# Somedaywilldo/BM-NAS

Measured on AMD Instinct MI355X. Metric: search-steps/sec (fwd+bwd of fusion hypernet) on MM-IMDB synthetic, higher is better.
Workload: dtype f32; 1 GPU; mmimdb fusion search, batch 128 per GPU x 1 GPU(s), N6 C192 L16 steps2 node_steps1 node_multiplier1, train mode, dropout 0.1/0.1(attn); inputs=(b, C, L) features, global_batch=128, per_gpu_batch=128, parallelism=dp1, mode=graph, step=fwd+bwd, one hipGraph replay

## Files before the change

### bm-nas_amd/csrc/arch_body.hpp

```cpp
#pragma once
#include "common.hpp"

namespace {

struct ArchPack {
  const float* a[BMNAS_MAX_PTRS];
  const float* b[BMNAS_MAX_PTRS];
  float* o[BMNAS_MAX_PTRS];
  int rows[BMNAS_MAX_PTRS], cols[BMNAS_MAX_PTRS];
  int n, n_shards;
  int64_t shard_stride;
};

__device__ __forceinline__ void arch_softmax_bwd_row(const ArchPack& P, int r, int lane) {
  const int col = lane & 3, sg = lane >> 2;
  for (int t = 0; t < P.n; ++t) {
    if (r < P.rows[t]) {
      const int cols = P.cols[t];
      float dw = 0.f, w = 0.f;
      if (col < cols) {
        const float* dwp = P.b[t] + r * cols + col;
        for (int sh = sg; sh < P.n_shards; sh += 16) dw += dwp[(int64_t)sh * P.shard_stride];
        w = P.a[t][r * cols + col];
      }
      dw = row_stride4_sum(dw);
      dw = xor16_sum(dw);
      dw = xor32_sum(dw);
      float dot = w * dw;
      dot += lane_xor1(dot);
      dot += lane_xor2(dot);
      if (sg == 0 && col < cols) P.o[t][r * cols + col] = w * (dw - dot);
      return;
    }
    r -= P.rows[t];
  }
}

inline int fill_arch_pack(ArchPack& P, const float* const* a, const float* const* dw, float* const* out,
                          const int* rows, const int* cols, int n, int backward, int n_shards,
                          int64_t shard_stride) {
  if (!a || !out || !rows || !cols || n < 1 || (backward && !dw) || n_shards < 1) return BMNAS_E_ARG;
  if (n > BMNAS_MAX_PTRS) return BMNAS_E_LIMIT;
  int total = 0;
  for (int t = 0; t < n; ++t) {
    if (!a[t] || !out[t] || rows[t] < 1 || cols[t] < 1 || cols[t] > 4 || (backward && !dw[t]))
      return BMNAS_E_ARG;
    P.a[t] = a[t];
    P.b[t] = backward ? dw[t] : nullptr;
    P.o[t] = out[t];
    P.rows[t] = rows[t];
    P.cols[t] = cols[t];
    total += rows[t];
  }
  P.n = n;
  P.n_shards = n_shards;
  P.shard_stride = shard_stride;
  return total;
}

}
```

### bm-nas_amd/csrc/bnmix.hip

```cpp
#include "common.hpp"
#include "../../include/bmnas_hip.h"
#include "arch_body.hpp"
#include "bn_fin.hpp"
#include "mix_common.hpp"
#include "mish.hpp"
#include <algorithm>
#include <cstdlib>

namespace {

constexpr float kEps = 1e-5f;
constexpr float kMomentum = 0.1f;

__global__ __launch_bounds__(256) void bn_finalize_k(const float* __restrict__ part, int n_part,
                                                     int b, int L, int M,
                                                     const float* __restrict__ bn_w,
                                                     const float* __restrict__ bn_b,
                                                     float* running_mean, float* running_var,
                                                     int64_t* nbt, int n_nbt, int training,
                                                     float* __restrict__ chan) {
  const int lane = threadIdx.x & 63;
  const int m = blockIdx.x * 4 + (threadIdx.x >> 6);
  if (m >= M) return;
  float mean, rstd;
// ... 1058 lines not shown
  float* Weff[kMaxFold];
  int n, M, C, blocks_per;
};

__device__ __forceinline__ void cell_prologue_body(const ArchPack& P, const FoldPack& F,
                                                   unsigned long long* step_counter,
                                                   const unsigned long long* step_span,
                                                   float* __restrict__ scrub, int64_t scrub4, const int bid,
                                                   const int nblocks) {
  const int nfb = F.n * F.blocks_per;
  for (int64_t i = (int64_t)bid * 256 + threadIdx.x; i < scrub4; i += (int64_t)nblocks * 256)
    st4_wt(scrub + 4 * i, make_float4(0.f, 0.f, 0.f, 0.f));
  if (step_counter != nullptr && bid == nblocks - 1 && threadIdx.x == 0)
    step_counter[0] += step_span[0];
  if (bid < nfb) {
    const int q = bid / F.blocks_per, bi = bid - q * F.blocks_per;
    const float* __restrict__ W = F.W[q];
    float* __restrict__ We = F.Weff[q];
    const int c4n = F.C / 4;
    const int total = F.M * c4n;
    for (int i = bi * 256 + threadIdx.x; i < total; i += F.blocks_per * 256) {
      const int m = i / c4n, c4 = i - m * c4n;
      const float* r = W + (int64_t)m * 2 * F.C + 4 * c4;
      st4_wt(We + (int64_t)m * F.C + 4 * c4, f4_add(ld4(r), ld4(r + F.C)));
    }
    return;
  }
  int r = (bid - nfb) * 256 + threadIdx.x;
  for (int t = 0; t < P.n; ++t) {
    if (r < P.rows[t]) {
      const int cols = P.cols[t];
      const float* a = P.a[t] + r * cols;
      float* o = P.o[t] + r * cols;
      float mx = a[0];
      for (int p = 1; p < cols; ++p) mx = fmaxf(mx, a[p]);
      float den = 0.f;
      for (int p = 0; p < cols; ++p) den += expf(a[p] - mx);
      for (int p = 0; p < cols; ++p) o[p] = expf(a[p] - mx) / den;
      return;
    }
    r -= P.rows[t];
  }
}

__global__ __launch_bounds__(256) void cell_prologue_k(ArchPack P, FoldPack F, unsigned long long* step_counter,
                                                       const unsigned long long* step_span,
                                                       float* __restrict__ scrub, int64_t scrub4) {
  cell_prologue_body(P, F, step_counter, step_span, scrub, scrub4, (int)blockIdx.x, (int)gridDim.x);
}

__device__ __forceinline__ float softmax2_col1(const float* a) {
  const float a0 = a[0], a1 = a[1];
  const float mx = fmaxf(a0, a1);
  const float e0 = expf(a0 - mx), e1 = expf(a1 - mx);
  return e1 / (e0 + e1);
}

struct PairArgs {
  PtrsIn xs;
  const float* alpha;
  const float* beta;
  float* out;
  float* out2;
  int64_t n4;
};

template <int NIN>
__global__ __launch_bounds__(256) void cell_prologue_pair_k(ArchPack P, FoldPack F, unsigned long long* step_counter,
                                                            const unsigned long long* step_span,
                                                            float* __restrict__ scrub, int64_t scrub4, int n_pro,
                                                            PairArgs A) {
  if ((int)blockIdx.x < n_pro) {
    cell_prologue_body(P, F, step_counter, step_span, scrub, scrub4, (int)blockIdx.x, n_pro);
    return;
  }
  float wj[NIN];
#pragma unroll
  for (int j = 0; j < NIN; ++j) wj[j] = softmax2_col1(A.alpha + 2 * j);
  const float s2 = softmax2_col1(A.beta) + softmax2_col1(A.beta + 2);
  const int64_t stride = (int64_t)(gridDim.x - n_pro) * 256;
  for (int64_t i = (int64_t)(blockIdx.x - n_pro) * 256 + threadIdx.x; i < A.n4; i += stride) {
    float4 v[NIN];
#pragma unroll
    for (int j = 0; j < NIN; ++j) v[j] = reinterpret_cast<const float4*>(A.xs.p[j])[i];
    float4 acc = f4_scale(v[0], wj[0]);
#pragma unroll
    for (int j = 1; j < NIN; ++j) {
      acc.x = fmaf(wj[j], v[j].x, acc.x);
      acc.y = fmaf(wj[j], v[j].y, acc.y);
      acc.z = fmaf(wj[j], v[j].z, acc.z);
      acc.w = fmaf(wj[j], v[j].w, acc.w);
    }
    st4_w0<0>(A.out + 4 * i, acc);
    st4_w0<0>(A.out2 + 4 * i, f4_scale(acc, s2));
  }
}

}

extern "C" int bmnas_version(void) { return 100; }

extern "C" int bmnas_bn_finalize(const float* part, int n_part, int b, int L, int M,
                                 const float* bn_w, const float* bn_b, float* running_mean,
                                 float* running_var, int64_t* num_batches_tracked, int n_nbt,
                                 int training, float* chan, void* stream) {
  if (!bn_w || !bn_b || !chan || M < 1 || b < 1 || L < 1) return BMNAS_E_ARG;
  if (training && (!part || n_part < 1 || b * L < 2)) return BMNAS_E_ARG;
  if (!training && (!running_mean || !running_var)) return BMNAS_E_ARG;
  hipLaunchKernelGGL(bn_finalize_k, dim3((M + 3) / 4), dim3(256), 0, (hipStream_t)stream, part,
                     n_part, b, L, M, bn_w, bn_b, running_mean, running_var, num_batches_tracked,
                     n_nbt, training, chan);
  BMNAS_CHECK_LAUNCH();
  return 0;
}

extern "C" int bmnas_node_mix_fwd_next(const float* x, const float* y, const float* p1, const float* U,
                                       float* chan, bmnas_bn_fin_t fin, const float* gamma, float* out,
                                       int b, int C, int L, bmnas_dropout_t drop_glu,
                                       bmnas_dropout_t drop_fc, const float* const* prev, int n_prev,
                                       const float* w, int w_stride, float* z_next, void* stream) {
  if (!x || !y || !p1 || !U || !chan || !gamma || !out || b < 0 || C < 1 || n_prev < 0) return BMNAS_E_ARG;
  if (L % 4 || L > 16) return BMNAS_E_SHAPE;
  if (n_prev > kMixPrev) return BMNAS_E_LIMIT;
  MixNextF N{};
  if (n_prev > 0) {
    if (!prev || !w || !z_next || w_stride < 1) return BMNAS_E_ARG;
    for (int j = 0; j < n_prev; ++j) {
// ... 618 lines not shown
```

### bm-nas_amd/csrc/common.hpp

```cpp
#pragma once
#include <hip/hip_runtime.h>
#include <stdint.h>

#define BMNAS_MAX_PTRS 16
#define BMNAS_WAVE 64

typedef __attribute__((ext_vector_type(4))) float f32x4;

struct PtrsIn { const float* p[BMNAS_MAX_PTRS]; };
struct PtrsOut { float* p[BMNAS_MAX_PTRS]; };

struct DropCfg {
  uint32_t thr;
  float scale;
  uint64_t seed;
  uint64_t offset;
  const uint64_t* step;
};

#define BMNAS_CHECK_LAUNCH()                         \
  do {                                               \
    hipError_t e__ = hipGetLastError();              \
    if (e__ != hipSuccess) return (int)e__;          \
  } while (0)
// ... 212 lines not shown
  float t = red[0];
#pragma unroll
  for (int k = 1; k < NW; ++k) t += red[k];
  v[0] = t;
  if (threadIdx.x == 0) {
#pragma unroll
    for (int i = 1; i < N; ++i) {
      float u = red[i * NW];
#pragma unroll
      for (int k = 1; k < NW; ++k) u += red[i * NW + k];
      v[i] = u;
    }
  }
}

template <typename T>
__device__ __forceinline__ T* sgpr_ptr(T* p) {
  asm volatile("" : "+s"(p));
  return p;
}
template <typename T, int N>
__device__ __forceinline__ T* pick_ptr(T* const (&arr)[N], int q) {
  T* p = sgpr_ptr(arr[0]);
#pragma unroll
  for (int qq = 1; qq < N; ++qq) {
    T* c = sgpr_ptr(arr[qq]);
    p = (q == qq) ? c : p;
  }
  return p;
}

__device__ __forceinline__ float4 ld4(const float* p) { return *reinterpret_cast<const float4*>(p); }
__device__ __forceinline__ void st4(float* p, float4 v) { *reinterpret_cast<float4*>(p) = v; }
__device__ __forceinline__ void st4_wt(float* p, float4 v) {
#if defined(BMNAS_NO_WT)
  *reinterpret_cast<float4*>(p) = v;
#else
  const f32x4 d = {v.x, v.y, v.z, v.w};
  asm volatile("global_store_dwordx4 %0, %1, off sc1\n\ts_nop 1" : : "v"(p), "v"(d) : "memory");
#endif
}

#ifndef BMNAS_WT_MASK
#define BMNAS_WT_MASK 0x29
#endif
template <int G>
__device__ __forceinline__ void st4_wtg(float* p, float4 v) {
  if constexpr ((BMNAS_WT_MASK >> G) & 1) st4_wt(p, v);
  else *reinterpret_cast<float4*>(p) = v;
}

#ifndef BMNAS_WT0_MASK
#define BMNAS_WT0_MASK 0x7FF
#endif
template <int K>
__device__ __forceinline__ void st4_w0(float* p, float4 v) {
  if constexpr ((BMNAS_WT0_MASK >> K) & 1) st4_wt(p, v);
  else *reinterpret_cast<float4*>(p) = v;
}

__device__ __forceinline__ void st16_wt(void* p, uint4 v) {
#if defined(BMNAS_NO_WT) || !((BMNAS_WT_MASK >> 5) & 1)
  *reinterpret_cast<uint4*>(p) = v;
#else
  typedef __attribute__((ext_vector_type(4))) unsigned u32x4_;
  const u32x4_ d = {v.x, v.y, v.z, v.w};
// ... 24 lines not shown
```

### bm-nas_amd/csrc/layernorm.hip

```cpp
#include "common.hpp"
#include <cstdlib>
#include "../../include/bmnas_hip.h"
#include "arch_body.hpp"

namespace {

constexpr float kEps = 1e-5f;

struct LnSrc {
  const float* p[4];
};
struct LnDst {
  float* p[4];
};

__device__ __forceinline__ const float* src_ptr(const LnSrc& s, int i4, int cl4, int sample) {
  const int q = i4 / cl4;
  const int off = i4 - q * cl4;
  return pick_ptr(s.p, q) + ((int64_t)sample * cl4 + off) * 4;
}

template <int VPT, int BS>
__global__ __launch_bounds__(BS) void cat_ln_fwd_k(LnSrc srcs, const float* __restrict__ resid,
                                                    const float* __restrict__ ln_w,
// ... 168 lines not shown
        float* a = d + ((int64_t)s * cl4 + off) * 4;
        st4_wtg<3>(a, (acc_mask & (1u << q)) ? f4_add(dx, ld4(a)) : dx);
      }
      if (dresid != nullptr) {
        float* a = dresid + ((int64_t)s * d4 + i) * 4;
        st4_wtg<3>(a, (acc_mask & (1u << 31)) ? f4_add(dx, ld4(a)) : dx);
      }
    }
  }
}


struct LnAffineProb {
  const float* g;
  const float* gscale;
  LnSrc srcs;
  const float* resid;
  const float* ln_w;
  const float* ln_b;
  const float* stats;
  float* dln_w;
  float* dln_b;
  int cl4, d4, relu, prenorm;
};

constexpr int kMaxLnProbs = 8;
struct LnAffineBatch {
  LnAffineProb p[kMaxLnProbs];
  int n, b, chunk;
};

__device__ __forceinline__ void ln_affine_body(const LnAffineProb& P, int b, int chunk, float4 (*red)[3][64]) {
  const int col = threadIdx.x & 63, sl = threadIdx.x >> 6;
  const int i = blockIdx.x * 64 + col;
  const bool active = i < P.d4;
  const float gs = (P.gscale != nullptr) ? P.gscale[0] : 1.f;
  float4 aw = make_float4(0.f, 0.f, 0.f, 0.f), ab = aw;
  if (active) {
    float4 w = make_float4(0.f, 0.f, 0.f, 0.f), bb = w;
    if (P.relu) {
      w = ld4(P.ln_w + (int64_t)i * 4);
      bb = ld4(P.ln_b + (int64_t)i * 4);
    }
    const int s_beg = blockIdx.y * chunk;
    int s_end = s_beg + chunk;
    if (s_end > b) s_end = b;
    for (int s = s_beg + sl; s < s_end; s += 4) {
      float4 x = ld4(src_ptr(P.srcs, i, P.cl4, s));
      float4 gy = f4_scale(ld4(P.g + ((int64_t)s * P.d4 + i) * 4), gs);
      float4 h = x;
      if (!P.prenorm) {
        if (P.resid != nullptr) x = f4_add(x, ld4(P.resid + ((int64_t)s * P.d4 + i) * 4));
        const float mean = P.stats[2 * s], rstd = P.stats[2 * s + 1];
        h = make_float4((x.x - mean) * rstd, (x.y - mean) * rstd, (x.z - mean) * rstd, (x.w - mean) * rstd);
      }
      if (P.relu) {
        if (h.x * w.x + bb.x <= 0.f) gy.x = 0.f;
        if (h.y * w.y + bb.y <= 0.f) gy.y = 0.f;
        if (h.z * w.z + bb.z <= 0.f) gy.z = 0.f;
        if (h.w * w.w + bb.w <= 0.f) gy.w = 0.f;
      }
      aw = f4_add(aw, f4_mul(gy, h));
      ab = f4_add(ab, gy);
    }
  }
  if (sl > 0) {
    red[0][sl - 1][col] = aw;
    red[1][sl - 1][col] = ab;
  }
  __syncthreads();
  if (sl == 0 && active) {
#pragma unroll
    for (int k = 0; k < 3; ++k) {
      aw = f4_add(aw, red[0][k][col]);
      ab = f4_add(ab, red[1][k][col]);
    }
    float* pw = P.dln_w + (int64_t)i * 4;
    float* pb = P.dln_b + (int64_t)i * 4;
    atomicAdd(pw + 0, aw.x); atomicAdd(pw + 1, aw.y); atomicAdd(pw + 2, aw.z); atomicAdd(pw + 3, aw.w);
    atomicAdd(pb + 0, ab.x); atomicAdd(pb + 1, ab.y); atomicAdd(pb + 2, ab.z); atomicAdd(pb + 3, ab.w);
  }
}

__global__ __launch_bounds__(256) void ln_affine_bwd_k(LnAffineBatch B) {
  __shared__ float4 red[2][3][64];
  const LnAffineProb& P = B.p[blockIdx.z];
  if ((int)blockIdx.x * 64 >= P.d4) return;
  ln_affine_body(P, B.b, B.chunk, red);
}

constexpr int kMaxSums = 2;
struct SumPack {
  const float* part[kMaxSums];
  float* out[kMaxSums];
  long long n4[kMaxSums];
  int n_chunk[kMaxSums];
  int n;
  int reps;
};

__global__ __launch_bounds__(256) void backward_epilogue_k(LnAffineBatch B, ArchPack A, int arch_rows, SumPack S) {
  __shared__ float4 red[2][3][64];
  if ((int)blockIdx.z > B.n) {
    const int k = (int)blockIdx.z - B.n - 1;
    const int i = k / S.reps, rep = k - i * S.reps;
    const long long per = (long long)gridDim.x * gridDim.y;
    const long long n4 = S.n4[i], wg = rep * per + (long long)blockIdx.y * gridDim.x + blockIdx.x;
    const float* __restrict__ part = S.part[i];
    for (long long e = wg * 256 + threadIdx.x; e < n4; e += (long long)S.reps * per * 256) {
      float4 t = ld4(part + 4 * e);
      for (int c = 1; c < S.n_chunk[i]; ++c) t = f4_add(t, ld4(part + 4 * (e + (long long)c * n4)));
      st4_wtg<3>(S.out[i] + 4 * e, t);
    }
    return;
  }
  if ((int)blockIdx.z == B.n) {
    const int r = ((int)blockIdx.y * (int)gridDim.x + (int)blockIdx.x) * 4 + (int)(threadIdx.x >> 6);
    if (r < arch_rows) arch_softmax_bwd_row(A, r, threadIdx.x & 63);
    return;
  }
  const LnAffineProb& P = B.p[blockIdx.z];
  if ((int)blockIdx.x * 64 >= P.d4) return;
  ln_affine_body(P, B.b, B.chunk, red);
}

inline int pick_vpt(int d4, int bs) {
  const int need = (d4 + bs - 1) / bs;
  if (need <= 1) return 1;
  if (need <= 2) return 2;
  if (need <= 3) return 3;
  if (need <= 4) return 4;
  if (need <= 8) return 8;
  if (need <= 16) return 16;
  return -1;
}

}

#define LN_DISPATCH(V, CALL)      \
  switch (V) {                    \
    case 1: CALL(1); break;       \
    case 2: CALL(2); break;       \
    case 3: CALL(3); break;       \
    case 4: CALL(4); break;       \
    case 8: CALL(8); break;       \
    case 16: CALL(16); break;     \
    default: return BMNAS_E_LIMIT; \
  }

extern "C" int bmnas_cat_ln_fwd(const float* const* srcs, int n_src, const float* resid,
// ... 195 lines not shown
```

### bm-nas_amd/csrc/lazyln.hip

```cpp
#include "common.hpp"
#include "../../include/bmnas_hip.h"
#include "bn_fin.hpp"
#include "lazy_ln.hpp"
#include "mix_common.hpp"

namespace {

__global__ __launch_bounds__(256) void node_mix_pre_fwd_k(
    const float* __restrict__ x, const float* __restrict__ y, const float* __restrict__ p1,
    const float* __restrict__ U, float* __restrict__ chan, BnFin fin, const float* __restrict__ gamma,
    const float* __restrict__ resid, const float* __restrict__ ln_w, const float* __restrict__ ln_b,
    float* __restrict__ pre, float* __restrict__ rec, float* __restrict__ prm, int b, int C, int L,
    DropCfg dglu, DropCfg dfc) {
  __shared__ float red[4];
  __shared__ float red5[2 * 4 * 5];
  extern __shared__ float fin_lds[];
  const int cl4 = C * L / 4, l4n = L / 4, M = 3 * C;
  const int part = blockIdx.x, smp = blockIdx.y, P = gridDim.x;
  STAMP(0, smp * P + part, 0);
  float* sc = fin_lds;
  float* sh = fin_lds + M;
  const int r0 = part * kLazyPart + threadIdx.x;
  const bool act = r0 < cl4;
  const int r = act ? r0 : cl4 - 1;
// ... 205 lines not shown
      float* d = dxs.p[j];
      if (d == nullptr) continue;
      float4 rr = f4_scale(g4, wj[j]);
      if (acc_mask & (1u << j)) {
        rr = f4_add(rr, j >= NIN - NLZ ? oldn[j - (NIN - NLZ) < 0 ? 0 : j - (NIN - NLZ)] : reinterpret_cast<float4*>(d)[i]);
      }
      st4_w0<9>(d + 4 * i, rr);
    }
  }
  STAMP(2, smp * P + part, 2);
  const int wave = threadIdx.x >> 6, lane = threadIdx.x & 63;
#pragma unroll
  for (int q = 0; q < NR; ++q) {
    if (!DOTS && q <= NIN) continue;
    const float sv = wave_sum(part_[q]);
    if (lane == 0) red[wave * NR + q] = sv;
  }
  __syncthreads();
  if ((int)threadIdx.x < NR + 1 && (DOTS || (int)threadIdx.x > NIN + 1)) {
    const int t = threadIdx.x;
    const int q = t <= NIN ? (t < NIN ? t : NIN) : t - 1;
    const float val = red[q] + red[NR + q] + red[2 * NR + q] + red[3 * NR + q];
    const int64_t shd = (int64_t)((smp * P + part) % dw_shards) * dw_shard_stride;
    if (t < NIN) atomicAdd(dw + shd + t * w_stride, val);
    else if (t <= NIN + 1) atomicAdd(dw2 + shd + (t - NIN) * w2_stride, val);
    else {
      const int u = t - (NIN + 2);
      Z.lnpart[u >> 1][((int64_t)smp * Z.stride[u >> 1] + part) * 2 + (u & 1)] = val;
    }
  }
  STAMP(2, smp * P + part, 3);
}

__global__ __launch_bounds__(256) void node_mix_lnp_bwd_k(
    const float* __restrict__ gy, const float* __restrict__ pre, const float* __restrict__ ln_w,
    const float* __restrict__ stats, const float* __restrict__ lnp0, int n0, const float* __restrict__ lnp1, int n1,
    float* __restrict__ gbuf, float* dresid, int acc_resid, const float* __restrict__ x,
    const float* __restrict__ y, const float* __restrict__ p1, const float* __restrict__ U,
    const float* __restrict__ chan, const float* __restrict__ gamma, float* dgamma, int dg_shards, int64_t dg_stride,
    float* dx, float* dy, uint32_t acc_mask, float* __restrict__ dV, float* bn_grad, float* __restrict__ bn_part,
    int b, int C, int L, int chunk, DropCfg dglu, DropCfg dfc) {
  __shared__ float red16[16];
  __shared__ float csum[3][6][64];
  const int cl4 = C * L / 4, l4n = L / 4, M = 3 * C;
  STAMP(3, blockIdx.y * gridDim.x + blockIdx.x, 0);
  const int col = threadIdx.x & 63, sl = threadIdx.x >> 6;
  const int r0 = blockIdx.x * 64 + col;
  const bool active = r0 < cl4;
  const int r = active ? r0 : cl4 - 1;
  const int c = r / l4n;
  const float g0 = gamma[0], g2 = gamma[2], g3 = gamma[3];
  const DropRt rglu = drop_begin(dglu), rfc = drop_begin(dfc);
  const ChanBn<3> bn = chan_load<3>(chan, M, C, c);
  const float4 lw = ld4(ln_w + (int64_t)r * 4);
  const float inv_d = 1.f / (float)(cl4 * 4);
  float dgam[4] = {0.f, 0.f, 0.f, 0.f};
  float sw[3] = {0.f, 0.f, 0.f}, sb[3] = {0.f, 0.f, 0.f};
  const int s_beg = blockIdx.y * chunk;
  int s_end = s_beg + chunk;
  if (s_end > b) s_end = b;
  const int np = n0 + n1;
  for (int s0 = s_beg; s0 < s_end; s0 += 4) {
    const int s_raw = s0 + sl;
    const bool on = active && s_raw < s_end;
    const int s = s_raw < s_end ? s_raw : s_end - 1;
    float q1 = 0.f, q2 = 0.f;
    for (int t = col; t < np; t += 64) {
      const float2 pp = t < n0 ? reinterpret_cast<const float2*>(lnp0)[(int64_t)s * n0 + t]
                               : reinterpret_cast<const float2*>(lnp1)[(int64_t)s * n1 + (t - n0)];
      q1 += pp.x;
      q2 += pp.y;
    }
    const float mean = stats[2 * s], rstd = stats[2 * s + 1];
    const int64_t e = ((int64_t)s * cl4 + r) * 4;
    const int64_t ub = ((int64_t)s * M) * L + (int64_t)r * 4;
    const float4 gyv = ld4(gy + e), prv = ld4(pre + e);
    const float4 ua = ld4(U + ub), ug = ld4(U + ub + (int64_t)C * L), uf = ld4(U + ub + (int64_t)2 * C * L);
    const float4 xv = ld4(x + e), yv = ld4(y + e), pv = ld4(p1 + e);
    float4 oldr = make_float4(0.f, 0.f, 0.f, 0.f), oldx = oldr, oldy = oldr;
    if (acc_resid) oldr = ld4(dresid + e);
    if (dx != nullptr && (acc_mask & 1u)) oldx = ld4(dx + e);
    if (dy != nullptr && (acc_mask & 2u)) oldy = ld4(dy + e);
    const float m1 = wave_sum(q1) * inv_d, m2 = wave_sum(q2) * inv_d;
    STAMP(3, blockIdx.y * gridDim.x + blockIdx.x, 1);
    if (on) {
      const float4 xh = make_float4((prv.x - mean) * rstd, (prv.y - mean) * rstd, (prv.z - mean) * rstd,
                                    (prv.w - mean) * rstd);
      float4 gv;
      gv.x = rstd * (gyv.x * lw.x - m1 - xh.x * m2);
      gv.y = rstd * (gyv.y * lw.y - m1 - xh.y * m2);
      gv.z = rstd * (gyv.z * lw.z - m1 - xh.z * m2);
      gv.w = rstd * (gyv.w * lw.w - m1 - xh.w * m2);
      if (gbuf != nullptr) st4_w0<6>(gbuf + e, gv);
      if (dresid != nullptr) st4_w0<6>(dresid + e, f4_add(gv, oldr));
      const float4 m2d = drop_mult4(rglu, (uint64_t)e), m3d = drop_mult4(rfc, (uint64_t)e);
      float4 da, dg, df;
      mix_bwd4<kMixAll>(g2, g3, gv, f4_add(xv, yv), pv, ua, ug, uf, m2d, m3d, bn, dgam, da, dg, df, sw, sb);
      st4_w0<6>(dV + ub, da);
      st4_w0<6>(dV + ub + (int64_t)C * L, dg);
      st4_w0<6>(dV + ub + (int64_t)2 * C * L, df);
      mix_dxy_store([](float* p, float4 v) { st4_w0<6>(p, v); }, dx, dy, e, gv, g0, oldx, oldy);
    }
  }
  STAMP(3, blockIdx.y * gridDim.x + blockIdx.x, 2);
  float cs[6];
#pragma unroll
  for (int k = 0; k < 3; ++k) {
    cs[k] = row_sum(sw[k], l4n);
    cs[3 + k] = row_sum(sb[k], l4n);
  }
  if (sl > 0) {
#pragma unroll
    for (int k = 0; k < 6; ++k) csum[sl - 1][k][col] = cs[k];
  }
#pragma unroll
  for (int q = 0; q < 4; ++q) dgam[q] = wave_sum(dgam[q]);
  if (col == 0) {
#pragma unroll
    for (int q = 0; q < 4; ++q) red16[q * 4 + sl] = dgam[q];
  }
  __syncthreads();
  if (sl == 0 && active && (r % l4n) == 0) {
#pragma unroll
    for (int k = 0; k < 6; ++k) cs[k] += csum[0][k][col] + csum[1][k][col] + csum[2][k][col];
    if (bn_part != nullptr) {
      float* row = bn_part + (int64_t)blockIdx.y * 2 * M;
#pragma unroll
      for (int k = 0; k < 3; ++k) {
        row[k * C + c] = cs[k];
        row[M + k * C + c] = cs[3 + k];
      }
    } else {
#pragma unroll
      for (int k = 0; k < 3; ++k) {
        atomicAdd(bn_grad + k * C + c, cs[k]);
// ... 134 lines not shown
  switch (n_in) {
    case 2: CALL2(2, 1); break;
    case 3: CALL(3); break;   case 4: CALL(4); break;   case 5: CALL(5); break;   case 6: CALL(6); break;
    case 7: CALL(7); break;   case 8: CALL(8); break;   case 9: CALL(9); break;   case 10: CALL(10); break;
    case 11: CALL(11); break; case 12: CALL(12); break; case 13: CALL(13); break; case 14: CALL(14); break;
    case 15: CALL(15); break;
    default: return BMNAS_E_LIMIT;
  }
#undef CALL
#undef CALL2
  BMNAS_CHECK_LAUNCH();
  return 0;
}

extern "C" int bmnas_node_mix_lnp_bwd(const float* g, const float* pre, const float* ln_w, const float* stats,
                                      const float* lnp0, int n0, const float* lnp1, int n1, float* g_in,
                                      float* dresid, int accumulate_resid, const float* x, const float* y,
                                      const float* p1, const float* U, const float* chan, const float* gamma,
                                      float* dgamma, int dgamma_shards, int64_t dgamma_shard_stride, float* dx,
                                      float* dy, uint32_t accumulate_mask, float* dV, float* bn_grad, int b, int C,
                                      int L, bmnas_dropout_t drop_glu, bmnas_dropout_t drop_fc, float* bn_part,
                                      void* stream) {
  if (!g || !pre || !ln_w || !stats || !x || !y || !p1 || !U || !chan || !gamma || !dV || !bn_grad || b < 0 ||
      C < 1 || dgamma_shards < 1 || n0 < 0 || n1 < 0 || (n0 > 0 && !lnp0) || (n1 > 0 && !lnp1) || n0 + n1 < 1)
    return BMNAS_E_ARG;
  if (accumulate_resid && !dresid) return BMNAS_E_ARG;
  if (!(L == 4 || L == 8 || L == 16)) return BMNAS_E_SHAPE;
  if (!bmnas_lazy_ln_ok(C, L)) return BMNAS_E_LIMIT;
  if (b == 0) return 0;
  const int cl4 = C * L / 4;
  int chunk = 4;
  while ((b + chunk - 1) / chunk > 64) chunk += 4;
  dim3 grid((cl4 + 63) / 64, (b + chunk - 1) / chunk);
  hipLaunchKernelGGL(node_mix_lnp_bwd_k, grid, dim3(256), 0, (hipStream_t)stream, g, pre, ln_w, stats, lnp0, n0,
                     lnp1, n1, g_in, dresid, accumulate_resid, x, y, p1, U, chan, gamma, dgamma, dgamma_shards,
                     dgamma_shard_stride, dx, dy, accumulate_mask, dV, bn_grad, bn_part, b, C, L, chunk,
                     to_cfg(drop_glu), to_cfg(drop_fc));
  BMNAS_CHECK_LAUNCH();
  if (bn_part != nullptr)
    return bmnas_sum_chunks(bn_part, bn_grad, (int)grid.y, (int64_t)6 * C, stream);
  return 0;
}

extern "C" int bmnas_node_mix_lnp_bwd_rows(int b) {
  if (b < 1) return BMNAS_E_ARG;
  int chunk = 4;
  while ((b + chunk - 1) / chunk > 64) chunk += 4;
  return (b + chunk - 1) / chunk;
}
```

### bm-nas_amd/csrc/mixsum.hip

```cpp
#include "common.hpp"
#include "../../include/bmnas_hip.h"

namespace {

template <int NIN>
__global__ __launch_bounds__(256) void mixsum_fwd_k(PtrsIn xs, const float* __restrict__ w,
                                                    int w_stride, float* __restrict__ out,
                                                    int64_t n4) {
  float wj[NIN];
#pragma unroll
  for (int j = 0; j < NIN; ++j) wj[j] = w[j * w_stride];
  const int64_t stride = (int64_t)gridDim.x * 256;
  for (int64_t i = (int64_t)blockIdx.x * 256 + threadIdx.x; i < n4; i += stride) {
    float4 v[NIN];
#pragma unroll
    for (int j = 0; j < NIN; ++j) v[j] = reinterpret_cast<const float4*>(xs.p[j])[i];
    float4 acc = f4_scale(v[0], wj[0]);
#pragma unroll
    for (int j = 1; j < NIN; ++j) {
      acc.x = fmaf(wj[j], v[j].x, acc.x);
      acc.y = fmaf(wj[j], v[j].y, acc.y);
      acc.z = fmaf(wj[j], v[j].z, acc.z);
      acc.w = fmaf(wj[j], v[j].w, acc.w);
    }
// ... 135 lines not shown
  for (int j = 0; j <= NIN; ++j) {
    float s = wave_sum(part[j]);
    if (lane == 0) red[wave * (NIN + 1) + j] = s;
  }
  __syncthreads();
  if (threadIdx.x <= NIN + 1) {
    const int j = threadIdx.x < NIN ? threadIdx.x : NIN;
    const float v = red[j] + red[NIN + 1 + j] + red[2 * (NIN + 1) + j] + red[3 * (NIN + 1) + j];
    const int64_t sh = (int64_t)(blockIdx.x % dw_shards) * dw_shard_stride;
    if (threadIdx.x < NIN) atomicAdd(dw + sh + j * w_stride, v);
    else atomicAdd(dw2 + sh + (threadIdx.x - NIN) * w2_stride, v);
  }
}

constexpr int kMaxMoreG = 2;
struct MoreG {
  const float* g[kMaxMoreG];
  const float* w[kMaxMoreG];
};

template <int NIN, int NX, bool DOTS = true>
__global__ __launch_bounds__(256) void mixsum_pair_bwd_x_k(PtrsIn xs, PtrsOut dxs,
                                                           const float* __restrict__ w, int w_stride,
                                                           const float* __restrict__ w2, int w2_stride,
                                                           const float* __restrict__ h,
                                                           const float* __restrict__ gh,
                                                           const float* __restrict__ gz,
                                                           const float* __restrict__ gz2, float* dw,
                                                           float* dw2, int dw_shards,
                                                           int64_t dw_shard_stride, uint32_t acc_mask,
                                                           MoreG X, int64_t n4) {
  __shared__ float red[4 * (NIN + 1)];
  float wj[NIN], wx[NX][NIN], part[NIN + 1];
#pragma unroll
  for (int j = 0; j < NIN; ++j) {
    wj[j] = w[j * w_stride];
    part[j] = 0.f;
#pragma unroll
    for (int t = 0; t < NX; ++t) wx[t][j] = X.w[t][j * w_stride];
  }
  part[NIN] = 0.f;
  const float s2 = w2[0] + w2[w2_stride];
  const int64_t stride = (int64_t)gridDim.x * 256;
  for (int64_t i = (int64_t)blockIdx.x * 256 + threadIdx.x; i < n4; i += stride) {
    const float4 zero4 = make_float4(0.f, 0.f, 0.f, 0.f);
    float4 z4 = reinterpret_cast<const float4*>(gz)[i];
    const float4 z2v = reinterpret_cast<const float4*>(gz2 != nullptr ? gz2 : gz)[i];
    float4 h4 = zero4;
    if constexpr (DOTS) h4 = reinterpret_cast<const float4*>(h)[i];
    const float4 ghv = reinterpret_cast<const float4*>(gh != nullptr ? gh : gz)[i];
    float4 gx[NX];
#pragma unroll
    for (int t = 0; t < NX; ++t) gx[t] = reinterpret_cast<const float4*>(X.g[t])[i];
    float4 v[NIN];
#pragma unroll
    for (int j = 0; j < NIN; ++j) {
      if constexpr (DOTS) v[j] = reinterpret_cast<const float4*>(xs.p[j])[i];
      else v[j] = zero4;
    }
    z4 = f4_add(z4, gz2 != nullptr ? z2v : zero4);
    const float4 g4 = f4_add(f4_scale(z4, s2), gh != nullptr ? ghv : zero4);
#pragma unroll
    for (int j = 0; j < NIN; ++j) part[j] += f4_dot(g4, v[j]);
    part[NIN] += f4_dot(z4, h4);
#pragma unroll
    for (int j = 0; j < NIN; ++j) {
      float* d = dxs.p[j];
      if (d == nullptr) continue;
      float4 r = f4_scale(g4, wj[j]);
#pragma unroll
      for (int t = 0; t < NX; ++t) {
        r.x = fmaf(wx[t][j], gx[t].x, r.x);
        r.y = fmaf(wx[t][j], gx[t].y, r.y);
        r.z = fmaf(wx[t][j], gx[t].z, r.z);
        r.w = fmaf(wx[t][j], gx[t].w, r.w);
      }
      if (acc_mask & (1u << j)) r = f4_add(r, reinterpret_cast<float4*>(d)[i]);
      st4_w0<10>(d + 4 * i, r);
    }
  }
  if constexpr (!DOTS) return;
  const int wave = threadIdx.x >> 6, lane = threadIdx.x & 63;
#pragma unroll
  for (int j = 0; j <= NIN; ++j) {
    float s = wave_sum(part[j]);
    if (lane == 0) red[wave * (NIN + 1) + j] = s;
  }
  __syncthreads();
  if (threadIdx.x <= NIN + 1) {
    const int j = threadIdx.x < NIN ? threadIdx.x : NIN;
    const float v = red[j] + red[NIN + 1 + j] + red[2 * (NIN + 1) + j] + red[3 * (NIN + 1) + j];
    const int64_t sh = (int64_t)(blockIdx.x % dw_shards) * dw_shard_stride;
    if (threadIdx.x < NIN) atomicAdd(dw + sh + j * w_stride, v);
    else atomicAdd(dw2 + sh + (threadIdx.x - NIN) * w2_stride, v);
  }
}

inline int grid_for(int64_t n4) {
  int64_t blocks = (n4 + 255) / 256;
  if (blocks > 2048) blocks = 2048;
  if (blocks < 1) blocks = 1;
  return (int)blocks;
}

}

#define MIXSUM_DISPATCH(N, CALL) \
  switch (N) {                   \
    case 1: CALL(1); break;      \
    case 2: CALL(2); break;      \
    case 3: CALL(3); break;      \
    case 4: CALL(4); break;      \
    case 5: CALL(5); break;      \
// ... 189 lines not shown
```

Baseline: 6970 steps/s.

## Hoist global loads ahead of dependent parameter loads across several backward kernels

```diff
diff --git a/bm-nas_amd/csrc/arch_body.hpp b/bm-nas_amd/csrc/arch_body.hpp
--- a/bm-nas_amd/csrc/arch_body.hpp
+++ b/bm-nas_amd/csrc/arch_body.hpp
@@ -14,26 +14,46 @@
 
 __device__ __forceinline__ void arch_softmax_bwd_row(const ArchPack& P, int r, int lane) {
   const int col = lane & 3, sg = lane >> 2;
-  for (int t = 0; t < P.n; ++t) {
-    if (r < P.rows[t]) {
-      const int cols = P.cols[t];
-      float dw = 0.f, w = 0.f;
-      if (col < cols) {
-        const float* dwp = P.b[t] + r * cols + col;
-        for (int sh = sg; sh < P.n_shards; sh += 16) dw += dwp[(int64_t)sh * P.shard_stride];
-        w = P.a[t][r * cols + col];
-      }
-      dw = row_stride4_sum(dw);
-      dw = xor16_sum(dw);
-      dw = xor32_sum(dw);
-      float dot = w * dw;
-      dot += lane_xor1(dot);
-      dot += lane_xor2(dot);
-      if (sg == 0 && col < cols) P.o[t][r * cols + col] = w * (dw - dot);
-      return;
-    }
-    r -= P.rows[t];
+  r = __builtin_amdgcn_readfirstlane(r);
+  int t = -1, rt = 0;
+#pragma unroll
+  for (int q = 0; q < BMNAS_MAX_PTRS; ++q) {
+    const bool here = t < 0 && q < P.n && r < P.rows[q];
+    t = here ? q : t;
+    rt = here ? r : rt;
+    r -= (t < 0 && q < P.n) ? P.rows[q] : 0;
   }
+  if (t < 0) return;
+  const int cols = P.cols[t];
+  const float* __restrict__ ap = P.a[t];
+  const float* __restrict__ bp = P.b[t];
+  float* __restrict__ op = P.o[t];
+  const bool live = col < cols;
+  const int at = rt * cols + (live ? col : 0);
+  const float* dwp = bp + at;
+  const int ns = P.n_shards;
+  const int64_t stride = P.shard_stride;
+  const float wv = ap[at];
+  const float v0 = dwp[(int64_t)(sg < ns ? sg : ns - 1) * stride];
+  const float v1 = dwp[(int64_t)(sg + 16 < ns ? sg + 16 : ns - 1) * stride];
+  float dw = 0.f;
+  if (live && sg < ns) dw += v0;
+  if (live && sg + 16 < ns) dw += v1;
+  for (int s0 = 32; s0 < ns; s0 += 32) {
+    const int sa = s0 + sg, sb = sa + 16;
+    const float va = dwp[(int64_t)(sa < ns ? sa : ns - 1) * stride];
+    const float vb = dwp[(int64_t)(sb < ns ? sb : ns - 1) * stride];
+    if (live && sa < ns) dw += va;
+    if (live && sb < ns) dw += vb;
+  }
+  const float w = live ? wv : 0.f;
+  dw = row_stride4_sum(dw);
+  dw = xor16_sum(dw);
+  dw = xor32_sum(dw);
+  float dot = w * dw;
+  dot += lane_xor1(dot);
+  dot += lane_xor2(dot);
+  if (sg == 0 && live) op[at] = w * (dw - dot);
 }
 
 inline int fill_arch_pack(ArchPack& P, const float* const* a, const float* const* dw, float* const* out,
diff --git a/bm-nas_amd/csrc/bnmix.hip b/bm-nas_amd/csrc/bnmix.hip
--- a/bm-nas_amd/csrc/bnmix.hip
+++ b/bm-nas_amd/csrc/bnmix.hip
@@ -1114,11 +1114,21 @@
       const int cols = P.cols[t];
       const float* a = P.a[t] + r * cols;
       float* o = P.o[t] + r * cols;
-      float mx = a[0];
-      for (int p = 1; p < cols; ++p) mx = fmaxf(mx, a[p]);
-      float den = 0.f;
-      for (int p = 0; p < cols; ++p) den += expf(a[p] - mx);
-      for (int p = 0; p < cols; ++p) o[p] = expf(a[p] - mx) / den;
+      float av[4];
+#pragma unroll
+      for (int p = 0; p < 4; ++p) av[p] = a[p < cols ? p : cols - 1];
+      float mx = av[0];
+#pragma unroll
+      for (int p = 1; p < 4; ++p) mx = p < cols ? fmaxf(mx, av[p]) : mx;
+      float ev[4], den = 0.f;
+#pragma unroll
+      for (int p = 0; p < 4; ++p) {
+        ev[p] = expf(av[p] - mx);
+        den = p < cols ? den + ev[p] : den;
+      }
+#pragma unroll
+      for (int p = 0; p < 4; ++p)
+        if (p < cols) o[p] = ev[p] / den;
       return;
     }
     r -= P.rows[t];
@@ -1156,15 +1166,18 @@
     cell_prologue_body(P, F, step_counter, step_span, scrub, scrub4, (int)blockIdx.x, n_pro);
     return;
   }
+  const int64_t stride = (int64_t)(gridDim.x - n_pro) * 256;
+  int64_t i = (int64_t)(blockIdx.x - n_pro) * 256 + threadIdx.x;
+  if (i >= A.n4) return;
+  float4 v[NIN];
+#pragma unroll
+  for (int j = 0; j < NIN; ++j) v[j] = reinterpret_cast<const float4*>(A.xs.p[j])[i];
+  __builtin_amdgcn_sched_barrier(0);
   float wj[NIN];
 #pragma unroll
   for (int j = 0; j < NIN; ++j) wj[j] = softmax2_col1(A.alpha + 2 * j);
   const float s2 = softmax2_col1(A.beta) + softmax2_col1(A.beta + 2);
-  const int64_t stride = (int64_t)(gridDim.x - n_pro) * 256;
-  for (int64_t i = (int64_t)(blockIdx.x - n_pro) * 256 + threadIdx.x; i < A.n4; i += stride) {
-    float4 v[NIN];
-#pragma unroll
-    for (int j = 0; j < NIN; ++j) v[j] = reinterpret_cast<const float4*>(A.xs.p[j])[i];
+  for (;;) {
     float4 acc = f4_scale(v[0], wj[0]);
 #pragma unroll
     for (int j = 1; j < NIN; ++j) {
@@ -1175,6 +1188,10 @@
     }
     st4_w0<0>(A.out + 4 * i, acc);
     st4_w0<0>(A.out2 + 4 * i, f4_scale(acc, s2));
+    i += stride;
+    if (i >= A.n4) break;
+#pragma unroll
+    for (int j = 0; j < NIN; ++j) v[j] = reinterpret_cast<const float4*>(A.xs.p[j])[i];
   }
 }
 
diff --git a/bm-nas_amd/csrc/common.hpp b/bm-nas_amd/csrc/common.hpp
--- a/bm-nas_amd/csrc/common.hpp
+++ b/bm-nas_amd/csrc/common.hpp
@@ -268,6 +268,9 @@
 
 __device__ __forceinline__ float4 ld4(const float* p) { return *reinterpret_cast<const float4*>(p); }
 __device__ __forceinline__ void st4(float* p, float4 v) { *reinterpret_cast<float4*>(p) = v; }
+__device__ __forceinline__ void pin4(float4& v) { asm volatile("" : "+v"(v.x), "+v"(v.y), "+v"(v.z), "+v"(v.w)); }
+__device__ __forceinline__ void pin1(float& v) { asm volatile("" : "+v"(v)); }
+
 __device__ __forceinline__ void st4_wt(float* p, float4 v) {
 #if defined(BMNAS_NO_WT)
   *reinterpret_cast<float4*>(p) = v;
diff --git a/bm-nas_amd/csrc/layernorm.hip b/bm-nas_amd/csrc/layernorm.hip
--- a/bm-nas_amd/csrc/layernorm.hip
+++ b/bm-nas_amd/csrc/layernorm.hip
@@ -224,36 +224,80 @@
 
 __device__ __forceinline__ void ln_affine_body(const LnAffineProb& P, int b, int chunk, float4 (*red)[3][64]) {
   const int col = threadIdx.x & 63, sl = threadIdx.x >> 6;
-  const int i = blockIdx.x * 64 + col;
-  const bool active = i < P.d4;
-  const float gs = (P.gscale != nullptr) ? P.gscale[0] : 1.f;
+  const int d4 = P.d4, cl4 = P.cl4;
+  const bool relu = P.relu != 0, prenorm = P.prenorm != 0;
+  const float* __restrict__ g = P.g;
+  const float* gscale = P.gscale;
+  const float* resid = P.resid;
+  const float* stats = P.stats;
+  const float* ln_w = P.ln_w;
+  const float* ln_b = P.ln_b;
+  float* dln_w = P.dln_w;
+  float* dln_b = P.dln_b;
+  const float* src[4] = {sgpr_ptr(P.srcs.p[0]), sgpr_ptr(P.srcs.p[1]), sgpr_ptr(P.srcs.p[2]), sgpr_ptr(P.srcs.p[3])};
+  const int i0 = blockIdx.x * 64 + col;
+  const bool active = i0 < d4;
+  const int i = active ? i0 : d4 - 1;
+  const int q = i / cl4;
+  const int off = i - q * cl4;
+  const float* xsrc = src[0];
+#pragma unroll
+  for (int qq = 1; qq < 4; ++qq) xsrc = (q == qq) ? src[qq] : xsrc;
+  const bool has_r = !prenorm && resid != nullptr, has_st = !prenorm;
+  const float* rp = has_r ? resid : g;
+  const float* sp = has_st ? stats : g;
+  const float4 w = ld4((relu ? ln_w : g) + (int64_t)i * 4);
+  const float4 bb = ld4((relu ? ln_b : g) + (int64_t)i * 4);
+  const float gsv = (gscale != nullptr ? gscale : g)[0];
   float4 aw = make_float4(0.f, 0.f, 0.f, 0.f), ab = aw;
-  if (active) {
-    float4 w = make_float4(0.f, 0.f, 0.f, 0.f), bb = w;
-    if (P.relu) {
-      w = ld4(P.ln_w + (int64_t)i * 4);
-      bb = ld4(P.ln_b + (int64_t)i * 4);
-    }
-    const int s_beg = blockIdx.y * chunk;
-    int s_end = s_beg + chunk;
-    if (s_end > b) s_end = b;
-    for (int s = s_beg + sl; s < s_end; s += 4) {
-      float4 x = ld4(src_ptr(P.srcs, i, P.cl4, s));
-      float4 gy = f4_scale(ld4(P.g + ((int64_t)s * P.d4 + i) * 4), gs);
-      float4 h = x;
-      if (!P.prenorm) {
-        if (P.resid != nullptr) x = f4_add(x, ld4(P.resid + ((int64_t)s * P.d4 + i) * 4));
-        const float mean = P.stats[2 * s], rstd = P.stats[2 * s + 1];
-        h = make_float4((x.x - mean) * rstd, (x.y - mean) * rstd, (x.z - mean) * rstd, (x.w - mean) * rstd);
-      }
-      if (P.relu) {
-        if (h.x * w.x + bb.x <= 0.f) gy.x = 0.f;
-        if (h.y * w.y + bb.y <= 0.f) gy.y = 0.f;
-        if (h.z * w.z + bb.z <= 0.f) gy.z = 0.f;
-        if (h.w * w.w + bb.w <= 0.f) gy.w = 0.f;
-      }
-      aw = f4_add(aw, f4_mul(gy, h));
-      ab = f4_add(ab, gy);
+  const int s_beg = blockIdx.y * chunk;
+  int s_end = s_beg + chunk;
+  if (s_end > b) s_end = b;
+  for (int sg = s_beg; sg < s_end; sg += 16) {
+    float4 xv[4], gv[4], rv[4];
+    float mean[4], rstd[4];
+#pragma unroll
+    for (int k = 0; k < 4; ++k) {
+      const int s_raw = sg + 4 * k + sl;
+      const int s = s_raw < s_end ? s_raw : s_end - 1;
+      xv[k] = ld4(xsrc + ((int64_t)s * cl4 + off) * 4);
+      gv[k] = ld4(g + ((int64_t)s * d4 + i) * 4);
+      rv[k] = ld4(rp + ((int64_t)s * d4 + i) * 4);
+      mean[k] = sp[2 * s];
+      rstd[k] = sp[2 * s + 1];
+    }
+    __builtin_amdgcn_sched_barrier(0);
+#pragma unroll
+    for (int k = 0; k < 4; ++k) {
+      pin4(xv[k]);
+      pin4(gv[k]);
+      pin4(rv[k]);
+      pin1(mean[k]);
+      pin1(rstd[k]);
+    }
+    float gs = gsv;
+    pin1(gs);
+    gs = gscale != nullptr ? gs : 1.f;
+#pragma unroll
+    for (int k = 0; k < 4; ++k) {
+      if (sg + 4 * k + sl < s_end) {
+        float4 x = xv[k];
+        float4 gy = f4_scale(gv[k], gs);
+        float4 h = x;
+        if (!prenorm) {
+          if (has_r) x = f4_add(x, rv[k]);
+          h = make_float4((x.x - mean[k]) * rstd[k], (x.y - mean[k]) * rstd[k], (x.z - mean[k]) * rstd[k],
+                          (x.w - mean[k]) * rstd[k]);
+        }
+        if (relu) {
+          if (h.x * w.x + bb.x <= 0.f) gy.x = 0.f;
+          if (h.y * w.y + bb.y <= 0.f) gy.y = 0.f;
+          if (h.z * w.z + bb.z <= 0.f) gy.z = 0.f;
+          if (h.w * w.w + bb.w <= 0.f) gy.w = 0.f;
+        }
+        aw = f4_add(aw, f4_mul(gy, h));
+        ab = f4_add(ab, gy);
+      }
     }
   }
   if (sl > 0) {
@@ -267,8 +311,8 @@
       aw = f4_add(aw, red[0][k][col]);
       ab = f4_add(ab, red[1][k][col]);
     }
-    float* pw = P.dln_w + (int64_t)i * 4;
-    float* pb = P.dln_b + (int64_t)i * 4;
+    float* pw = dln_w + (int64_t)i * 4;
+    float* pb = dln_b + (int64_t)i * 4;
     atomicAdd(pw + 0, aw.x); atomicAdd(pw + 1, aw.y); atomicAdd(pw + 2, aw.z); atomicAdd(pw + 3, aw.w);
     atomicAdd(pb + 0, ab.x); atomicAdd(pb + 1, ab.y); atomicAdd(pb + 2, ab.z); atomicAdd(pb + 3, ab.w);
   }
@@ -299,15 +343,29 @@
     const long long per = (long long)gridDim.x * gridDim.y;
     const long long n4 = S.n4[i], wg = rep * per + (long long)blockIdx.y * gridDim.x + blockIdx.x;
     const float* __restrict__ part = S.part[i];
-    for (long long e = wg * 256 + threadIdx.x; e < n4; e += (long long)S.reps * per * 256) {
-      float4 t = ld4(part + 4 * e);
-      for (int c = 1; c < S.n_chunk[i]; ++c) t = f4_add(t, ld4(part + 4 * (e + (long long)c * n4)));
-      st4_wtg<3>(S.out[i] + 4 * e, t);
+    float* __restrict__ out = S.out[i];
+    const int nc = S.n_chunk[i];
+    const long long step = (long long)S.reps * per * 256;
+    for (long long e = wg * 256 + threadIdx.x; e < n4; e += step) {
+      float4 t = make_float4(0.f, 0.f, 0.f, 0.f);
+      for (int c0 = 0; c0 < nc; c0 += 4) {
+        float4 v[4];
+#pragma unroll
+        for (int k = 0; k < 4; ++k) v[k] = ld4(part + 4 * (e + (long long)(c0 + k < nc ? c0 + k : nc - 1) * n4));
+        __builtin_amdgcn_sched_barrier(0);
+#pragma unroll
+        for (int k = 0; k < 4; ++k) pin4(v[k]);
+#pragma unroll
+        for (int k = 0; k < 4; ++k)
+          if (c0 + k < nc) t = (c0 + k == 0) ? v[k] : f4_add(t, v[k]);
+      }
+      st4_wtg<3>(out + 4 * e, t);
     }
     return;
   }
   if ((int)blockIdx.z == B.n) {
-    const int r = ((int)blockIdx.y * (int)gridDim.x + (int)blockIdx.x) * 4 + (int)(threadIdx.x >> 6);
+    const int r = ((int)blockIdx.y * (int)gridDim.x + (int)blockIdx.x) * 4 +
+                  __builtin_amdgcn_readfirstlane((int)(threadIdx.x >> 6));
     if (r < arch_rows) arch_softmax_bwd_row(A, r, threadIdx.x & 63);
     return;
   }
diff --git a/bm-nas_amd/csrc/lazyln.hip b/bm-nas_amd/csrc/lazyln.hip
--- a/bm-nas_amd/csrc/lazyln.hip
+++ b/bm-nas_amd/csrc/lazyln.hip
@@ -261,6 +261,69 @@
   STAMP(2, smp * P + part, 3);
 }
 
+template <int NPL>
+struct LnpTrip {
+  float2 pp[NPL > 0 ? NPL : 1];
+  float2 st;
+  float4 gy, pre, ua, ug, uf, x, y, p1, oldr, oldx, oldy;
+  int64_t e, ub;
+  bool on;
+};
+
+template <int NPL>
+__device__ __forceinline__ LnpTrip<NPL> lnp_issue(
+    int s0, int s_end, int sl, int col, bool active, int r, int cl4, int M, int C, int L,
+    const float* __restrict__ gy, const float* __restrict__ pre, const float* __restrict__ stats,
+    const float* __restrict__ lnp0, int n0, const float* __restrict__ lnp1, int n1, const float* oldr_p,
+    const float* oldx_p, const float* oldy_p, const float* __restrict__ x, const float* __restrict__ y,
+    const float* __restrict__ p1, const float* __restrict__ U) {
+  LnpTrip<NPL> t;
+  const int s_raw = s0 + sl;
+  t.on = active && s_raw < s_end;
+  const int s = s_raw < s_end ? s_raw : s_end - 1;
+  const int np = n0 + n1;
+  if constexpr (NPL > 0) {
+#pragma unroll
+    for (int k = 0; k < NPL; ++k) {
+      const int t0 = col + 64 * k;
+      const int tc = t0 < np ? t0 : np - 1;
+      const float2* src = tc < n0 ? reinterpret_cast<const float2*>(lnp0) + ((int64_t)s * n0 + tc)
+                                  : reinterpret_cast<const float2*>(lnp1) + ((int64_t)s * n1 + (tc - n0));
+      t.pp[k] = *src;
+    }
+  } else {
+    float q1 = 0.f, q2 = 0.f;
+#pragma unroll 1
+    for (int u0 = 0; u0 < np; u0 += 64) {
+      const int u = u0 + col;
+      const int uc = u < np ? u : np - 1;
+      const float2 pp = uc < n0 ? reinterpret_cast<const float2*>(lnp0)[(int64_t)s * n0 + uc]
+                                : reinterpret_cast<const float2*>(lnp1)[(int64_t)s * n1 + (uc - n0)];
+      if (u < np) {
+        q1 += pp.x;
+        q2 += pp.y;
+      }
+    }
+    t.pp[0] = make_float2(q1, q2);
+  }
+  t.st = make_float2(stats[2 * s], stats[2 * s + 1]);
+  t.e = ((int64_t)s * cl4 + r) * 4;
+  t.ub = ((int64_t)s * M) * L + (int64_t)r * 4;
+  t.gy = ld4(gy + t.e);
+  t.pre = ld4(pre + t.e);
+  t.ua = ld4(U + t.ub);
+  t.ug = ld4(U + t.ub + (int64_t)C * L);
+  t.uf = ld4(U + t.ub + (int64_t)2 * C * L);
+  t.x = ld4(x + t.e);
+  t.y = ld4(y + t.e);
+  t.p1 = ld4(p1 + t.e);
+  t.oldr = ld4(oldr_p + t.e);
+  t.oldx = ld4(oldx_p + t.e);
+  t.oldy = ld4(oldy_p + t.e);
+  return t;
+}
+
+template <int NPL>
 __global__ __launch_bounds__(256) void node_mix_lnp_bwd_k(
     const float* __restrict__ gy, const float* __restrict__ pre, const float* __restrict__ ln_w,
     const float* __restrict__ stats, const float* __restrict__ lnp0, int n0, const float* __restrict__ lnp1, int n1,
@@ -278,10 +341,6 @@
   const bool active = r0 < cl4;
   const int r = active ? r0 : cl4 - 1;
   const int c = r / l4n;
-  const float g0 = gamma[0], g2 = gamma[2], g3 = gamma[3];
-  const DropRt rglu = drop_begin(dglu), rfc = drop_begin(dfc);
-  const ChanBn<3> bn = chan_load<3>(chan, M, C, c);
-  const float4 lw = ld4(ln_w + (int64_t)r * 4);
   const float inv_d = 1.f / (float)(cl4 * 4);
   float dgam[4] = {0.f, 0.f, 0.f, 0.f};
   float sw[3] = {0.f, 0.f, 0.f}, sb[3] = {0.f, 0.f, 0.f};
@@ -289,47 +348,65 @@
   int s_end = s_beg + chunk;
   if (s_end > b) s_end = b;
   const int np = n0 + n1;
-  for (int s0 = s_beg; s0 < s_end; s0 += 4) {
-    const int s_raw = s0 + sl;
-    const bool on = active && s_raw < s_end;
-    const int s = s_raw < s_end ? s_raw : s_end - 1;
+  const bool use_r = acc_resid != 0, use_x = dx != nullptr && (acc_mask & 1u), use_y = dy != nullptr && (acc_mask & 2u);
+  const float* oldr_p = use_r ? dresid : gy;
+  const float* oldx_p = use_x ? dx : gy;
+  const float* oldy_p = use_y ? dy : gy;
+  const float4 zero4 = make_float4(0.f, 0.f, 0.f, 0.f);
+  LnpTrip<NPL> t;
+  if constexpr (NPL > 0)
+    t = lnp_issue<NPL>(s_beg, s_end, sl, col, active, r, cl4, M, C, L, gy, pre, stats, lnp0, n0, lnp1, n1, oldr_p,
+                       oldx_p, oldy_p, x, y, p1, U);
+  const float4 lw = ld4(ln_w + (int64_t)r * 4);
+  const ChanBn<3> bn = chan_load<3>(chan, M, C, c);
+  __builtin_amdgcn_sched_barrier(0);
+  const float g0 = gamma[0], g2 = gamma[2], g3 = gamma[3];
+  const DropRt rglu = drop_begin(dglu), rfc = drop_begin(dfc);
+  for (int s0 = s_beg;;) {
+    if constexpr (NPL == 0)
+      t = lnp_issue<NPL>(s0, s_end, sl, col, active, r, cl4, M, C, L, gy, pre, stats, lnp0, n0, lnp1, n1, oldr_p,
+                         oldx_p, oldy_p, x, y, p1, U);
     float q1 = 0.f, q2 = 0.f;
-    for (int t = col; t < np; t += 64) {
-      const float2 pp = t < n0 ? reinterpret_cast<const float2*>(lnp0)[(int64_t)s * n0 + t]
-                               : reinterpret_cast<const float2*>(lnp1)[(int64_t)s * n1 + (t - n0)];
-      q1 += pp.x;
-      q2 += pp.y;
-    }
-    const float mean = stats[2 * s], rstd = stats[2 * s + 1];
-    const int64_t e = ((int64_t)s * cl4 + r) * 4;
-    const int64_t ub = ((int64_t)s * M) * L + (int64_t)r * 4;
-    const float4 gyv = ld4(gy + e), prv = ld4(pre + e);
-    const float4 ua = ld4(U + ub), ug = ld4(U + ub + (int64_t)C * L), uf = ld4(U + ub + (int64_t)2 * C * L);
-    const float4 xv = ld4(x + e), yv = ld4(y + e), pv = ld4(p1 + e);
-    float4 oldr = make_float4(0.f, 0.f, 0.f, 0.f), oldx = oldr, oldy = oldr;
-    if (acc_resid) oldr = ld4(dresid + e);
-    if (dx != nullptr && (acc_mask & 1u)) oldx = ld4(dx + e);
-    if (dy != nullptr && (acc_mask & 2u)) oldy = ld4(dy + e);
+    if constexpr (NPL > 0) {
+#pragma unroll
+      for (int k = 0; k < NPL; ++k) {
+        if (col + 64 * k < np) {
+          q1 += t.pp[k].x;
+          q2 += t.pp[k].y;
+        }
+      }
+    } else {
+      q1 = t.pp[0].x;
+      q2 = t.pp[0].y;
+    }
+    const float mean = t.st.x, rstd = t.st.y;
     const float m1 = wave_sum(q1) * inv_d, m2 = wave_sum(q2) * inv_d;
     STAMP(3, blockIdx.y * gridDim.x + blockIdx.x, 1);
-    if (on) {
-      const float4 xh = make_float4((prv.x - mean) * rstd, (prv.y - mean) * rstd, (prv.z - mean) * rstd,
-                                    (prv.w - mean) * rstd);
+    if (t.on) {
+      const int64_t e = t.e, ub = t.ub;
+      const float4 xh = make_float4((t.pre.x - mean) * rstd, (t.pre.y - mean) * rstd, (t.pre.z - mean) * rstd,
+                                    (t.pre.w - mean) * rstd);
       float4 gv;
-      gv.x = rstd * (gyv.x * lw.x - m1 - xh.x * m2);
-      gv.y = rstd * (gyv.y * lw.y - m1 - xh.y * m2);
-      gv.z = rstd * (gyv.z * lw.z - m1 - xh.z * m2);
-      gv.w = rstd * (gyv.w * lw.w - m1 - xh.w * m2);
+      gv.x = rstd * (t.gy.x * lw.x - m1 - xh.x * m2);
+      gv.y = rstd * (t.gy.y * lw.y - m1 - xh.y * m2);
+      gv.z = rstd * (t.gy.z * lw.z - m1 - xh.z * m2);
+      gv.w = rstd * (t.gy.w * lw.w - m1 - xh.w * m2);
       if (gbuf != nullptr) st4_w0<6>(gbuf + e, gv);
-      if (dresid != nullptr) st4_w0<6>(dresid + e, f4_add(gv, oldr));
+      if (dresid != nullptr) st4_w0<6>(dresid + e, f4_add(gv, use_r ? t.oldr : zero4));
       const float4 m2d = drop_mult4(rglu, (uint64_t)e), m3d = drop_mult4(rfc, (uint64_t)e);
       float4 da, dg, df;
-      mix_bwd4<kMixAll>(g2, g3, gv, f4_add(xv, yv), pv, ua, ug, uf, m2d, m3d, bn, dgam, da, dg, df, sw, sb);
+      mix_bwd4<kMixAll>(g2, g3, gv, f4_add(t.x, t.y), t.p1, t.ua, t.ug, t.uf, m2d, m3d, bn, dgam, da, dg, df, sw, sb);
       st4_w0<6>(dV + ub, da);
       st4_w0<6>(dV + ub + (int64_t)C * L, dg);
       st4_w0<6>(dV + ub + (int64_t)2 * C * L, df);
-      mix_dxy_store([](float* p, float4 v) { st4_w0<6>(p, v); }, dx, dy, e, gv, g0, oldx, oldy);
-    }
+      mix_dxy_store([](float* p, float4 v) { st4_w0<6>(p, v); }, dx, dy, e, gv, g0, use_x ? t.oldx : zero4,
+                    use_y ? t.oldy : zero4);
+    }
+    s0 += 4;
+    if (s0 >= s_end) break;
+    if constexpr (NPL > 0)
+      t = lnp_issue<NPL>(s0, s_end, sl, col, active, r, cl4, M, C, L, gy, pre, stats, lnp0, n0, lnp1, n1, oldr_p,
+                         oldx_p, oldy_p, x, y, p1, U);
   }
   STAMP(3, blockIdx.y * gridDim.x + blockIdx.x, 2);
   float cs[6];
@@ -530,10 +607,20 @@
   int chunk = 4;
   while ((b + chunk - 1) / chunk > 64) chunk += 4;
   dim3 grid((cl4 + 63) / 64, (b + chunk - 1) / chunk);
-  hipLaunchKernelGGL(node_mix_lnp_bwd_k, grid, dim3(256), 0, (hipStream_t)stream, g, pre, ln_w, stats, lnp0, n0,
-                     lnp1, n1, g_in, dresid, accumulate_resid, x, y, p1, U, chan, gamma, dgamma, dgamma_shards,
-                     dgamma_shard_stride, dx, dy, accumulate_mask, dV, bn_grad, bn_part, b, C, L, chunk,
-                     to_cfg(drop_glu), to_cfg(drop_fc));
+  const int npl = (n0 + n1 + 63) / 64;
+#define CALL(N)                                                                                                     \
+  hipLaunchKernelGGL(node_mix_lnp_bwd_k<N>, grid, dim3(256), 0, (hipStream_t)stream, g, pre, ln_w, stats, lnp0, n0, \
+                     lnp1, n1, g_in, dresid, accumulate_resid, x, y, p1, U, chan, gamma, dgamma, dgamma_shards,     \
+                     dgamma_shard_stride, dx, dy, accumulate_mask, dV, bn_grad, bn_part, b, C, L, chunk,            \
+                     to_cfg(drop_glu), to_cfg(drop_fc))
+  switch (npl) {
+    case 1: CALL(1); break;
+    case 2: CALL(2); break;
+    case 3: CALL(3); break;
+    case 4: CALL(4); break;
+    default: CALL(0); break;
+  }
+#undef CALL
   BMNAS_CHECK_LAUNCH();
   if (bn_part != nullptr)
     return bmnas_sum_chunks(bn_part, bn_grad, (int)grid.y, (int64_t)6 * C, stream);
diff --git a/bm-nas_amd/csrc/mixsum.hip b/bm-nas_amd/csrc/mixsum.hip
--- a/bm-nas_amd/csrc/mixsum.hip
+++ b/bm-nas_amd/csrc/mixsum.hip
@@ -191,53 +191,82 @@
                                                            MoreG X, int64_t n4) {
   __shared__ float red[4 * (NIN + 1)];
   float wj[NIN], wx[NX][NIN], part[NIN + 1];
-#pragma unroll
-  for (int j = 0; j < NIN; ++j) {
-    wj[j] = w[j * w_stride];
-    part[j] = 0.f;
-#pragma unroll
-    for (int t = 0; t < NX; ++t) wx[t][j] = X.w[t][j * w_stride];
-  }
-  part[NIN] = 0.f;
-  const float s2 = w2[0] + w2[w2_stride];
+  struct Trip {
+    float4 z4, z2v, h4, ghv, gx[NX], v[NIN];
+  };
+  const float4 zero4 = make_float4(0.f, 0.f, 0.f, 0.f);
+  auto issue = [&](int64_t i) {
+    Trip t;
+    t.z4 = reinterpret_cast<const float4*>(gz)[i];
+    t.z2v = reinterpret_cast<const float4*>(gz2 != nullptr ? gz2 : gz)[i];
+    t.h4 = zero4;
+    if constexpr (DOTS) t.h4 = reinterpret_cast<const float4*>(h)[i];
+    t.ghv = reinterpret_cast<const float4*>(gh != nullptr ? gh : gz)[i];
+#pragma unroll
+    for (int k = 0; k < NX; ++k) t.gx[k] = reinterpret_cast<const float4*>(X.g[k])[i];
+#pragma unroll
+    for (int j = 0; j < NIN; ++j) {
+      if constexpr (DOTS) t.v[j] = reinterpret_cast<const float4*>(xs.p[j])[i];
+      else t.v[j] = zero4;
+    }
+    return t;
+  };
   const int64_t stride = (int64_t)gridDim.x * 256;
-  for (int64_t i = (int64_t)blockIdx.x * 256 + threadIdx.x; i < n4; i += stride) {
-    const float4 zero4 = make_float4(0.f, 0.f, 0.f, 0.f);
-    float4 z4 = reinterpret_cast<const float4*>(gz)[i];
-    const float4 z2v = reinterpret_cast<const float4*>(gz2 != nullptr ? gz2 : gz)[i];
-    float4 h4 = zero4;
-    if constexpr (DOTS) h4 = reinterpret_cast<const float4*>(h)[i];
-    const float4 ghv = reinterpret_cast<const float4*>(gh != nullptr ? gh : gz)[i];
-    float4 gx[NX];
-#pragma unroll
-    for (int t = 0; t < NX; ++t) gx[t] = reinterpret_cast<const float4*>(X.g[t])[i];
-    float4 v[NIN];
-#pragma unroll
-    for (int j = 0; j < NIN; ++j) {
-      if constexpr (DOTS) v[j] = reinterpret_cast<const float4*>(xs.p[j])[i];
-      else v[j] = zero4;
-    }
-    z4 = f4_add(z4, gz2 != nullptr ? z2v : zero4);
-    const float4 g4 = f4_add(f4_scale(z4, s2), gh != nullptr ? ghv : zero4);
-#pragma unroll
-    for (int j = 0; j < NIN; ++j) part[j] += f4_dot(g4, v[j]);
-    part[NIN] += f4_dot(z4, h4);
+  int64_t i = (int64_t)blockIdx.x * 256 + threadIdx.x;
+  bool live = i < n4;
+  auto weights = [&]() {
+#pragma unroll
+    for (int j = 0; j < NIN; ++j) {
+      wj[j] = w[j * w_stride];
+#pragma unroll
+      for (int k = 0; k < NX; ++k) wx[k][j] = X.w[k][j * w_stride];
+    }
+    return w2[0] + w2[w2_stride];
+  };
+#pragma unroll
+  for (int j = 0; j <= NIN; ++j) part[j] = 0.f;
+  auto finish = [&](const Trip& t, int64_t i, float s2, bool on) {
+    const float4 z4 = f4_add(t.z4, gz2 != nullptr ? t.z2v : zero4);
+    const float4 g4 = f4_add(f4_scale(z4, s2), gh != nullptr ? t.ghv : zero4);
+#pragma unroll
+    for (int j = 0; j < NIN; ++j) {
+      const float dj = f4_dot(g4, t.v[j]);
+      part[j] += on ? dj : 0.f;
+    }
+    const float dh = f4_dot(z4, t.h4);
+    part[NIN] += on ? dh : 0.f;
 #pragma unroll
     for (int j = 0; j < NIN; ++j) {
       float* d = dxs.p[j];
-      if (d == nullptr) continue;
+      if (d == nullptr || !on) continue;
       float4 r = f4_scale(g4, wj[j]);
 #pragma unroll
-      for (int t = 0; t < NX; ++t) {
-        r.x = fmaf(wx[t][j], gx[t].x, r.x);
-        r.y = fmaf(wx[t][j], gx[t].y, r.y);
-        r.z = fmaf(wx[t][j], gx[t].z, r.z);
-        r.w = fmaf(wx[t][j], gx[t].w, r.w);
+      for (int k = 0; k < NX; ++k) {
+        r.x = fmaf(wx[k][j], t.gx[k].x, r.x);
+        r.y = fmaf(wx[k][j], t.gx[k].y, r.y);
+        r.z = fmaf(wx[k][j], t.gx[k].z, r.z);
+        r.w = fmaf(wx[k][j], t.gx[k].w, r.w);
       }
       if (acc_mask & (1u << j)) r = f4_add(r, reinterpret_cast<float4*>(d)[i]);
       st4_w0<10>(d + 4 * i, r);
     }
-  }
+  };
+  Trip t = issue(live ? i : n4 - 1);
+  __builtin_amdgcn_sched_barrier(0);
+  const float s2 = weights();
+  __builtin_amdgcn_sched_barrier(0);
+  pin4(t.z4);
+  pin4(t.z2v);
+  pin4(t.ghv);
+  if constexpr (DOTS) pin4(t.h4);
+#pragma unroll
+  for (int k = 0; k < NX; ++k) pin4(t.gx[k]);
+  if constexpr (DOTS) {
+#pragma unroll
+    for (int j = 0; j < NIN; ++j) pin4(t.v[j]);
+  }
+  finish(t, i, s2, live);
+  for (i += stride; i < n4; i += stride) finish(issue(i), i, s2, true);
   if constexpr (!DOTS) return;
   const int wave = threadIdx.x >> 6, lane = threadIdx.x & 63;
 #pragma unroll
```

Result: faster. 7302 steps/s, median of 6 (+4.8%).
